# bacpop/sparrowhawk

Hardware: AMD Instinct MI355X
Metric: Gbases/s assembled, k=31 150bp reads (higher is better)
Workload: dtype u64

## Files before the change

sparrowhawk_amd/csrc/graph_part.h:

```cpp
#pragma once

struct MinScan {
    Nt32State first, last;
    uint32_t h_first, h_last;
    uint32_t min_wo_first;
    uint32_t min_wo_last;
    __device__ __forceinline__ uint32_t min_all() const { return min(min_wo_first, h_first); }
};

template <int W> __device__ __forceinline__ uint32_t km_base(const Kmer<W> &x, int k, int j) {
    return km_bits2<W>(x, 2 * (k - 1 - j));
}

template <int W> __device__ __forceinline__ MinScan km_min_scan(const Kmer<W> &x, int k, int gm) {
    MinScan r;
    Nt32State nt{0, 0};
    for (int j = 0; j < gm; j++) nt32_init_step(nt, km_base<W>(x, k, j), (unsigned)j);
    r.first = nt; r.h_first = nt32_canonical(nt);
    r.min_wo_first = 0xFFFFFFFFu; r.min_wo_last = r.h_first;
    const int w = k - gm + 1;
    uint32_t h = r.h_first;
    for (int q = 1; q < w; q++) {
        nt32_roll(nt, km_base<W>(x, k, q - 1), km_base<W>(x, k, q + gm - 1), (unsigned)gm);
        h = nt32_canonical(nt);
// ... 128 lines not shown
}

__global__ __launch_bounds__(1024) void k_gp_scan(uint32_t *__restrict__ gp_cnt , uint32_t GP,
                                                  unsigned long long *__restrict__ off, uint32_t *__restrict__ msk,
                                                  uint32_t *__restrict__ roff, unsigned long long *__restrict__ total) {
    constexpr uint32_t PER = 16, CH = 1024 * PER;
    __shared__ uint32_t lc[CH + CH / PER];
    __shared__ unsigned long long run_off[1024];
    __shared__ uint32_t run_roff[1024];
    __shared__ unsigned long long wsum[16];
    __shared__ uint32_t rsum[16];
    const int lane = threadIdx.x & 63, wid = threadIdx.x >> 6;
    unsigned long long carry = 0; uint32_t rcarry = 0;
    for (uint32_t c0 = 0; c0 < GP; c0 += CH) {
#pragma unroll
        for (uint32_t j = 0; j < PER; j++) {
            const uint32_t e = j * 1024u + threadIdx.x, p = c0 + e;
            lc[e + (e >> 4)] = p < GP ? gp_cnt[p] : 0u;
        }
#pragma unroll
        for (uint32_t j = 0; j < PER; j++) {
            const uint32_t p = c0 + j * 1024u + threadIdx.x;
            if (p < GP) gp_cnt[p] = 0u;
        }
        __syncthreads();
        unsigned long long my = 0; uint32_t myr = 0;
#pragma unroll
        for (uint32_t j = 0; j < PER; j++) {
            const uint32_t c = lc[threadIdx.x * (PER + 1u) + j];
            uint32_t sz = gp_table_size(c);
            if (c0 + threadIdx.x * PER + j >= GP) sz = 0;
            my += sz; myr += c;
        }
        unsigned long long incl = my; uint32_t rincl = myr;
        for (int o = 1; o < 64; o <<= 1) {
            const unsigned long long u = __shfl_up(incl, o); const uint32_t ru = (uint32_t)__shfl_up((int)rincl, o);
            if (lane >= o) { incl += u; rincl += ru; }
        }
        if (lane == 63) { wsum[wid] = incl; rsum[wid] = rincl; }
        __syncthreads();
        unsigned long long base = carry + incl - my; uint32_t rbase = rcarry + rincl - myr;
        for (int w = 0; w < wid; w++) { base += wsum[w]; rbase += rsum[w]; }
        run_off[threadIdx.x] = base; run_roff[threadIdx.x] = rbase;
        __syncthreads();
#pragma unroll 4
        for (uint32_t j = 0; j < PER; j++) {
            const uint32_t e = j * 1024u + threadIdx.x, p = c0 + e;
            const uint32_t c = lc[e + (e >> 4)];
            uint32_t sz = gp_table_size(c);
            if (p >= GP) sz = 0;
            uint32_t si = sz, ci = c;
#pragma unroll
            for (int o = 1; o < 16; o <<= 1) {
                const uint32_t u = (uint32_t)__shfl_up((int)si, o), v = (uint32_t)__shfl_up((int)ci, o);
                if ((lane & 15) >= o) { si += u; ci += v; }
            }
            if (p < GP) { off[p] = run_off[e >> 4] + (si - sz); msk[p] = sz - 1u; roff[p] = run_roff[e >> 4] + (ci - c); }
        }
        for (int w = 0; w < 16; w++) { carry += wsum[w]; rcarry += rsum[w]; }
        __syncthreads();
    }
    if (threadIdx.x == 0) { *total = carry; roff[GP] = rcarry; }
}

__global__ __launch_bounds__(256) void k_gp_rows(const uint32_t *__restrict__ gp_of, uint32_t n,
                                                 const uint32_t *__restrict__ roff, uint32_t *__restrict__ cursor,
                                                 uint32_t *__restrict__ rows) {
    const int lane = threadIdx.x & 63;
    const uint32_t stride = gridDim.x * blockDim.x;
    const uint32_t n_round = (n + stride - 1) / stride * stride;
    for (uint32_t i = blockIdx.x * blockDim.x + threadIdx.x; i < n_round; i += stride) {
        const uint32_t p = i < n ? gp_of[i] : 0xFFFFFFFFu;
        const bool valid = p != 0xFFFFFFFFu;
        unsigned long long todo = __ballot(valid);
        int my_leader = lane; uint32_t rank = 0, gsize = 0;
        while (todo) {
            const int leader = __ffsll((long long)todo) - 1;
            const uint32_t lp = (uint32_t)__shfl((int)p, leader);
            const unsigned long long same = __ballot(p == lp) & todo;
            if (valid && p == lp) { my_leader = leader; rank = (uint32_t)__popcll(same & ((1ull << lane) - 1ull)); gsize = (uint32_t)__popcll(same); }
            todo &= ~same;
        }
        const uint32_t ro = valid ? roff[p] : 0u;
        uint32_t base = 0;
        if (valid && lane == my_leader) base = atomicAdd(&cursor[p], gsize);
        base = (uint32_t)__shfl((int)base, my_leader);
        if (valid) rows[ro + base + rank] = i;
    }
}

template <int W>
__global__ __launch_bounds__(256) void k_regroup_rows(KeyArr<W> keys, const uint32_t *__restrict__ cnt, const uint32_t *__restrict__ gp_of,
                                                      uint32_t *__restrict__ rows, uint32_t n, KeyArr<W> out_keys,
                                                      uint32_t *__restrict__ out_cnt, uint32_t *__restrict__ out_gp_of) {
    for (uint32_t r = blockIdx.x * blockDim.x + threadIdx.x; r < n; r += gridDim.x * blockDim.x) {
        const uint32_t i = rows[r];
        out_keys.store(r, keys.load(i));
        out_cnt[r] = cnt[i];
        out_gp_of[r] = gp_of[i];
        rows[r] = r;
    }
}

template <int W>
__device__ __forceinline__ uint32_t gt_lookup_in(const GraphTable &gt, const KeyArr<W> &keys, const Kmer<W> &q,
                                                 uint32_t p) {
    const uint64_t h = gt_hash<W>(q);
    const uint32_t fp = (uint32_t)(h >> 32);
    const unsigned long long base = gt.off[p];
    const uint32_t mask = gt.msk[p];
    uint32_t slot = (uint32_t)h & mask;
    for (uint32_t t = 0; t <= mask; t++) {
        const uint64_t e = gt.e[base + slot];
        if (e == EMPTY64) return NIL;
        if ((uint32_t)(e >> 32) == fp) {
            const uint32_t idx = (uint32_t)e;
            if (km_eq<W>(keys.load(idx), q)) return idx;
        }
        slot = (slot + 1) & mask;
    }
    return NIL;
}
template <int W>
__device__ __forceinline__ uint32_t gt_lookup(const GraphTable &gt, const KeyArr<W> &keys, const Kmer<W> &q, int k) {
    return gt_lookup_in<W>(gt, keys, q, gt_partition_of<W>(gt, q, k));
}

static constexpr uint32_t ADJ_LDS_SLOTS = 2048;
static constexpr uint32_t NB_MULTI = 0xFFFFFFFEu;
static constexpr uint32_t ADJ_LDS_SLOTS_RANGES = 4096;
static constexpr int ADJ_THREADS_RANGES = 512;

struct GpRows {
    const uint32_t *roff;
    const uint32_t *cnt;
    const uint32_t *rows;
    __device__ __forceinline__ uint32_t begin(uint32_t P) const { return roff[P]; }
    __device__ __forceinline__ uint32_t end(uint32_t P) const { return cnt ? roff[P] + cnt[P] : roff[P + 1]; }
    __device__ __forceinline__ uint32_t row(uint32_t r) const { return rows ? rows[r] : r; }
};

template <int W>
__device__ __forceinline__ Kmer<W> adj_candidate(const Kmer<W> &x, const Kmer<W> &rx, int k, uint32_t j, bool &o) {
    Kmer<W> s = x, rr = rx;
    if (j < 4) { km_push_back<W>(s, j, k); km_push_front<W>(rr, 3u - j, k); }
    else { km_push_front<W>(s, j - 4u, k); km_push_back<W>(rr, 3u - (j - 4u), k); }
    o = km_less<W>(rr, s);
    Kmer<W> c;
#pragma unroll
    for (int w = 0; w < W; w++) c.w[w] = o ? rr.w[w] : s.w[w];
    return c;
}

template <int W, uint32_t SLOTS, int NT>
__global__ __launch_bounds__(NT) void k_graph_local(KeyArr<W> keys, int k, GraphTable gt, GpRows gr,
                                                    uint8_t *__restrict__ adj, uint32_t *__restrict__ nb,
                                                    unsigned long long *__restrict__ queries, uint32_t *__restrict__ qcnt,
                                                    uint32_t *__restrict__ overflow, uint32_t lds_slots ,
                                                    uint8_t *__restrict__ alive, uint32_t *__restrict__ row_bits, uint32_t lowmask) {
    const unsigned gm = (unsigned)gt.gm;
    __shared__ uint2 lut[16];
    __shared__ uint64_t tab[SLOTS];
    __shared__ uint32_t tabi[W == 1 ? SLOTS : 1];
    __shared__ uint32_t q_fill;
    const uint32_t P = blockIdx.x;
    const bool ranges = gr.cnt != nullptr;
    const uint32_t r0 = gr.begin(P), r1 = gr.end(P);
    const uint32_t pmask = gt.msk[P];
    const bool in_lds = pmask < lds_slots;
    uint64_t *gtab = gt.e + gt.off[P];
    nt32_fill_lut(lut, gm);
    const Nt32State all_a = nt32_all_a(gt.gm);
    if (threadIdx.x == 0) q_fill = 0;
    constexpr bool KEYS_IN_LDS = W == 1;
    for (uint32_t t = threadIdx.x; t <= pmask; t += blockDim.x) {
        if (in_lds) tab[t] = EMPTY64;
        if (!in_lds || KEYS_IN_LDS) gtab[t] = EMPTY64;
    }
    __syncthreads();
    constexpr int KEEP = 4;
    static_assert(SLOTS <= 2u * KEEP * NT, "a partition whose table fits the LDS keeps its rows in registers");
    const bool keep = W <= 2 && (r1 - r0) <= (uint32_t)KEEP * NT;
    static_assert(KEEP == 4, "kept rows are four named registers");
    const uint32_t rt = r0 + threadIdx.x;
    const uint32_t i0 = (keep && rt < r1) ? gr.row(rt) : NIL, i1 = (keep && rt + NT < r1) ? gr.row(rt + NT) : NIL;
    const uint32_t i2 = (keep && rt + 2 * NT < r1) ? gr.row(rt + 2 * NT) : NIL, i3 = (keep && rt + 3 * NT < r1) ? gr.row(rt + 3 * NT) : NIL;
    const Kmer<W> k0 = i0 != NIL ? keys.load(i0) : km_zero<W>(), k1 = i1 != NIL ? keys.load(i1) : km_zero<W>();
    const Kmer<W> k2 = i2 != NIL ? keys.load(i2) : km_zero<W>(), k3 = i3 != NIL ? keys.load(i3) : km_zero<W>();
    auto kept_i = [=](uint32_t q) { return q == 0 ? i0 : (q == 1 ? i1 : (q == 2 ? i2 : i3)); };
    auto kept_key = [=](uint32_t q) {
        Kmer<W> r;
#pragma unroll
        for (int w = 0; w < W; w++) r.w[w] = q == 0 ? k0.w[w] : (q == 1 ? k1.w[w] : (q == 2 ? k2.w[w] : k3.w[w]));
        return r;
    };
    for (uint32_t r = r0 + threadIdx.x, q = 0; r < r1; r += blockDim.x, q++) {
        const uint32_t i = keep ? kept_i(q) : gr.row(r);
        const Kmer<W> key = keep ? kept_key(q) : keys.load(i);
        const uint64_t h = gt_hash<W>(key);
        const uint64_t entry = (h & 0xFFFFFFFF00000000ull) | (uint64_t)i;
        uint32_t slot = (uint32_t)h & pmask;
        bool done = false;
        for (uint32_t t = 0; t <= pmask; t++) {
            if (in_lds && KEYS_IN_LDS) {
                if (atomicCAS((unsigned long long *)&tab[slot], (unsigned long long)EMPTY64, (unsigned long long)key.w[0]) == EMPTY64) {
                    tabi[slot] = i; gtab[slot] = entry; done = true; break;
                }
            } else {
                unsigned long long *cell = in_lds ? (unsigned long long *)&tab[slot] : (unsigned long long *)&gtab[slot];
                if (atomicCAS(cell, (unsigned long long)EMPTY64, (unsigned long long)entry) == EMPTY64) { done = true; break; }
            }
            slot = (slot + 1) & pmask;
        }
        if (!done) *overflow = 1;
    }
    __syncthreads();
    if (ranges && threadIdx.x == NT - 1 && r1 > r0) {
        bool st = r0 == 0u;
        if (!st) st = ((km_min_scan_lut<W>(keys.load(r0 - 1u), k, gt.gm, lut, all_a).min_all() ^ P) & lowmask) != 0u;
        if (st) atomicOr(&row_bits[r0 >> 5], 1u << (r0 & 31u));
    }
    if (in_lds && !KEYS_IN_LDS) for (uint32_t t = threadIdx.x; t <= pmask; t += blockDim.x) gtab[t] = tab[t];
    {
        uint8_t *occ = gt.occ + (gt.off[P] >> 3);
        for (uint32_t t8 = threadIdx.x; t8 <= (pmask >> 3); t8 += blockDim.x) {
            uint32_t bits = 0;
#pragma unroll
            for (uint32_t b = 0; b < 8; b++) {
                const uint64_t e = in_lds ? tab[8u * t8 + b] : __hip_atomic_load(&gtab[8u * t8 + b], __ATOMIC_RELAXED, __HIP_MEMORY_SCOPE_AGENT);
                bits |= (e != EMPTY64 ? 1u : 0u) << b;
            }
            occ[t8] = (uint8_t)bits;
        }
    }
    if (SHK_DBG(gt.dbg) == 1) { if (threadIdx.x == 0) qcnt[P] = 0; return; }
    unsigned long long *myq = queries + 8ull * r0;
    const int lane = threadIdx.x & 63;
    const uint32_t n_rows = r1 - r0;
    const uint32_t n_round = (n_rows + blockDim.x - 1) / blockDim.x * blockDim.x;
    for (uint32_t rr_ = threadIdx.x, q = 0; rr_ < n_round; rr_ += blockDim.x, q++) {
        const bool act = rr_ < n_rows;
        const uint32_t i = act ? (keep ? kept_i(q) : gr.row(r0 + rr_)) : 0u;
        Kmer<W> x = km_zero<W>(), rx = km_zero<W>();
        MinScan ms{};
        uint32_t out_b = 0, last_b = 0;
        if (act) {
            x = keep ? kept_key(q) : keys.load(i);
            rx = km_revcomp<W>(x, k);
            if (gt.scan) {
                const uint2 a = gt.scan[i], b = gt.scan[(size_t)gt.scan_n + i], c = gt.scan[2 * (size_t)gt.scan_n + i];
                ms.first.fh = a.x; ms.first.rh = a.y; ms.last.fh = b.x; ms.last.rh = b.y; ms.min_wo_first = c.x; ms.min_wo_last = c.y;
                ms.h_first = min(a.x, a.y); ms.h_last = min(b.x, b.y);
            } else
            if (SHK_DBG(gt.dbg) != 2) ms = km_min_scan_lut<W>(x, k, gt.gm, lut, all_a);
            if (ranges && ((ms.min_all() & gt.gp_mask) != P)) *overflow = 2u;
            out_b = km_base<W>(x, k, k - (int)gm);
            last_b = km_base<W>(x, k, (int)gm - 1);
        }
        uint32_t a = 0, n_out = 0, n_in = 0, u_out = NIL, u_in = NIL;
#pragma unroll
        for (uint32_t j = 0; j < 8; j++) {
            bool remote = false; uint32_t p = 0, xowner = 0; bool cross = false;
            if (act) {
                const uint32_t hmin = j < 4 ? min(ms.min_wo_first, nt32_next_hash_lut(ms.last, out_b, j, lut))
                                            : min(ms.min_wo_last, nt32_prev_hash_lut(ms.first, j - 4u, last_b, lut));
                p = hmin & gt.gp_mask;
                if (gt.world > 1) { xowner = gt.owner_of(hmin); cross = xowner != gt.rank; }
                remote = cross || p != P || !in_lds;
                if (SHK_DBG(gt.dbg) == 3) remote = false;
                if (SHK_DBG(gt.dbg) == 4 && remote) { remote = false; }
                else if (!remote && SHK_DBG(gt.dbg) != 3) {
                    bool o; const Kmer<W> c = adj_candidate<W>(x, rx, k, j, o);
                    const uint64_t h = gt_hash<W>(c);
                    const uint32_t fp = (uint32_t)(h >> 32);
                    uint32_t slot = (uint32_t)h & pmask, idx = NIL;
                    for (uint32_t t = 0; t <= pmask; t++) {
                        const uint64_t e = tab[slot];
                        if (e == EMPTY64) break;
                        if constexpr (KEYS_IN_LDS) { if (e == c.w[0]) { idx = tabi[slot]; break; } }
                        else if ((uint32_t)(e >> 32) == fp && km_eq<W>(keys.load((uint32_t)e), c)) { idx = (uint32_t)e; break; }
                        slot = (slot + 1) & pmask;
                    }
                    (void)fp;
                    if (idx != NIL) {
                        a |= 1u << j;
                        if (j < 4) { n_out++; u_out = idx * 2u + (o ? 1u : 0u); }
                        else { n_in++; u_in = idx * 2u + (o ? 0u : 1u); }
                    }
                }
            }
            const unsigned long long m = __ballot(remote);
            if (m) {
                uint32_t base = 0;
                if (lane == 0) base = atomicAdd(&q_fill, (uint32_t)__popcll(m));
                base = (uint32_t)__shfl((int)base, 0);
                if (remote) myq[base + (uint32_t)__popcll(m & ((1ull << lane) - 1ull))] =
                    (unsigned long long)i | ((unsigned long long)j << 32) | ((unsigned long long)p << 35) |
                    (cross ? (1ull << 63) | ((unsigned long long)xowner << 52) : 0ull);
            }
        }
        if (act) {
            adj[i] = (uint8_t)a;
            if (alive) alive[i] = 1;
            uint2 v;
            v.x = n_out == 0 ? NIL : (n_out == 1 ? u_out : NB_MULTI);
            v.y = n_in == 0 ? NIL : (n_in == 1 ? u_in : NB_MULTI);
            *reinterpret_cast<uint2 *>(nb + 2ull * i) = v;
        }
    }
    __syncthreads();
    if (threadIdx.x == 0) qcnt[P] = q_fill;
}

template <int W>
__global__ __launch_bounds__(256) void k_graph_remote(KeyArr<W> keys, int k, GraphTable gt, GpRows gr,
                                                      const unsigned long long *__restrict__ queries,
                                                      const uint32_t *__restrict__ qcnt,
                                                      uint8_t *__restrict__ adj, uint32_t *__restrict__ nb) {
    const uint32_t P = blockIdx.x;
    const unsigned long long *myq = queries + 8ull * gr.begin(P);
    const uint32_t nq = qcnt[P];
    constexpr int U = W <= 2 ? 4 : (W <= 4 ? 2 : 1);
    for (uint32_t t0 = threadIdx.x; t0 < nq; t0 += blockDim.x * U) {
        unsigned long long q[U]; bool live[U];
#pragma unroll
        for (int u = 0; u < U; u++) {
            const uint32_t t = t0 + (uint32_t)u * blockDim.x;
            q[u] = t < nq ? myq[t] : ~0ull;
            live[u] = !(q[u] >> 63);
        }
        Kmer<W> x[U]; unsigned long long tbase[U]; uint32_t tmask[U];
#pragma unroll
        for (int u = 0; u < U; u++) {
            const uint32_t i = (uint32_t)q[u], p = (uint32_t)(q[u] >> 35) & 0x1FFFFu;
            x[u] = live[u] ? keys.load(i) : km_zero<W>();
            tbase[u] = live[u] ? gt.off[p] : 0ull;
            tmask[u] = live[u] ? gt.msk[p] : 0u;
        }
        Kmer<W> c[U]; bool o[U]; uint32_t fp[U], slot[U]; uint64_t e[U];
#pragma unroll
        for (int u = 0; u < U; u++) {
            const uint32_t j = (uint32_t)(q[u] >> 32) & 7u;
            const Kmer<W> rx = km_revcomp<W>(x[u], k);
            c[u] = adj_candidate<W>(x[u], rx, k, j, o[u]);
            const uint64_t h = gt_hash<W>(c[u]);
            fp[u] = (uint32_t)(h >> 32); slot[u] = (uint32_t)h & tmask[u];
        }
        bool taken[U];
#pragma unroll
        for (int u = 0; u < U; u++) {
            const unsigned long long s = tbase[u] + slot[u];
            taken[u] = live[u] && ((gt.occ[s >> 3] >> (s & 7u)) & 1u);
        }
#pragma unroll
        for (int u = 0; u < U; u++) e[u] = taken[u] ? gt.e[tbase[u] + slot[u]] : EMPTY64;
        Kmer<W> cand[U]; bool want[U];
#pragma unroll
        for (int u = 0; u < U; u++) {
            want[u] = e[u] != EMPTY64 && (uint32_t)(e[u] >> 32) == fp[u];
            cand[u] = want[u] ? keys.load((uint32_t)e[u]) : km_zero<W>();
        }
#pragma unroll
        for (int u = 0; u < U; u++) {
            if (!live[u]) continue;
            uint32_t idx = NIL;
            if (want[u] && km_eq<W>(cand[u], c[u])) idx = (uint32_t)e[u];
            else if (e[u] != EMPTY64) {
                uint32_t s = (slot[u] + 1u) & tmask[u];
                for (uint32_t t = 1; t <= tmask[u]; t++) {
                    const uint64_t ee = gt.e[tbase[u] + s];
                    if (ee == EMPTY64) break;
                    if ((uint32_t)(ee >> 32) == fp[u] && km_eq<W>(keys.load((uint32_t)ee), c[u])) { idx = (uint32_t)ee; break; }
                    s = (s + 1u) & tmask[u];
                }
            }
            if (idx == NIL) continue;
            const uint32_t i = (uint32_t)q[u], j = (uint32_t)(q[u] >> 32) & 7u;
            atomicOr((uint32_t *)adj + (i >> 2), (1u << j) << (8 * (i & 3u)));
            const uint32_t v = j < 4 ? idx * 2u + (o[u] ? 1u : 0u) : idx * 2u + (o[u] ? 0u : 1u);
            uint32_t *dst = nb + 2ull * i + (j < 4 ? 0 : 1);
            if (atomicCAS(dst, NIL, v) != NIL) atomicExch(dst, NB_MULTI);
        }
    }
}

__device__ __forceinline__ uint32_t rev4(uint32_t n) {
    return ((n & 1) << 3) | ((n & 2) << 1) | ((n & 4) >> 1) | ((n & 8) >> 3);
}
__device__ __forceinline__ uint32_t outmask_of(uint32_t adjbyte, uint32_t o) {
    return o ? rev4(adjbyte >> 4) : (adjbyte & 15u);
}

template <int W> struct Graph {
    KeyArr<W> keys;
    const uint32_t *cnt;
    uint8_t *adj;
    GraphTable gt;
    const uint32_t *nb;
    int k;
    uint32_t n;
    uint32_t xref = 0;
    __device__ __forceinline__ uint32_t outmask(uint32_t v) const { return outmask_of(adj[v >> 1], v & 1); }
    __device__ __forceinline__ uint32_t outdeg(uint32_t v) const { return __popc(outmask(v)); }
    __device__ __forceinline__ uint32_t indeg(uint32_t v) const { return __popc(outmask(v ^ 1)); }
    __device__ __forceinline__ Kmer<W> seq(uint32_t v) const {
        Kmer<W> x = keys.load(v >> 1);
        return (v & 1) ? km_revcomp<W>(x, k) : x;
    }
    __device__ __forceinline__ uint32_t follow(uint32_t v, uint32_t b) const {
        Kmer<W> s = seq(v);
        km_push_back<W>(s, b, k);
        int o; Kmer<W> c = km_canonical<W>(s, k, o);
        uint32_t idx = gt_lookup<W>(gt, keys, c, k);
        return idx == NIL ? NIL : idx * 2 + (uint32_t)o;
    }
    __device__ __forceinline__ uint32_t only_out(uint32_t v) const {
        const uint32_t c = nb[v];
        if (c < NB_MULTI) return c;
        return follow(v, (uint32_t)__ffs((int)outmask(v)) - 1);
    }
};

struct TipRec { uint32_t start, junction, len, next; unsigned long long sum; };

template <int W>
__global__ __launch_bounds__(256) void k_tip_candidates(Graph<W> g, const uint8_t *__restrict__ alive,
                                                        uint32_t *__restrict__ cand,
                                                        unsigned int *__restrict__ n_cand,
                                                        uint2 *__restrict__ init_tip_head ,
                                                        uint8_t *__restrict__ init_mark ) {
    const int lane = threadIdx.x & 63;
    const uint32_t stride = gridDim.x * blockDim.x;
    const uint32_t n_round = (g.n + stride - 1) / stride * stride;
    for (uint32_t i = blockIdx.x * blockDim.x + threadIdx.x; i < n_round; i += stride) {
        uint32_t a = 0; bool al = false;
        if (i < g.n) {
            a = g.adj[i]; al = alive[i] != 0;
            if (init_tip_head) { uint2 nil; nil.x = NIL; nil.y = NIL; init_tip_head[i] = nil; init_mark[i] = 0; }
        }
#pragma unroll
        for (uint32_t o = 0; o < 2; o++) {
            const bool p = al && __popc(outmask_of(a, o ^ 1u)) == 0 && __popc(outmask_of(a, o)) == 1;
            const unsigned long long m = __ballot(p);
            if (!m) continue;
            unsigned int base = 0;
            if (lane == 0) base = atomicAdd(n_cand, (unsigned int)__popcll(m));
            base = __shfl(base, 0);
            if (p) cand[base + __popcll(m & ((1ull << lane) - 1ull))] = 2u * i + o;
        }
    }
}

template <int W>
__global__ __launch_bounds__(256) void k_tip_walk(Graph<W> g, const uint32_t *__restrict__ cand,
                                                  const unsigned int *__restrict__ n_cand_p, TipRec *__restrict__ tips,
                                                  unsigned int *__restrict__ n_tips,
                                                  uint32_t *__restrict__ tip_head) {
    const uint32_t T_TIP = 2u * (uint32_t)g.k;
    const uint32_t n_cand = *n_cand_p;
    for (uint32_t c = blockIdx.x * blockDim.x + threadIdx.x; c < n_cand; c += gridDim.x * blockDim.x) {
        const uint32_t v = cand[c];
        uint32_t cur = v, len = 1, J = NIL;
        unsigned long long sum = g.cnt[v >> 1];
        uint32_t a_cur = g.adj[cur >> 1], nb_cur = g.nb[cur];
        for (;;) {
            const uint32_t om = outmask_of(a_cur, cur & 1u);
            if (__popc(om) != 1) break;
            const uint32_t n = nb_cur < NB_MULTI ? nb_cur : g.follow(cur, (uint32_t)__ffs((int)om) - 1u);
            if (n == NIL) break;
            const uint32_t a_n = g.adj[n >> 1], nb_n = g.nb[n], c_n = g.cnt[n >> 1];
            if (__popc(outmask_of(a_n, (n & 1u) ^ 1u)) >= 2) { J = n; break; }
            len++; sum += c_n; cur = n; a_cur = a_n; nb_cur = nb_n;
            if (len > T_TIP) break;
        }
        if (J == NIL || len > T_TIP) continue;
        const uint32_t t = atomicAdd(n_tips, 1u);
        TipRec r; r.start = v; r.junction = J; r.len = len; r.sum = sum;
        r.next = atomicExch(&tip_head[J], t);
        tips[t] = r;
    }
}

template <int W>
__global__ __launch_bounds__(256) void k_tip_decide(Graph<W> g, const TipRec *__restrict__ tips,
                                                    const unsigned int *__restrict__ n_tips_p,
                                                    const uint32_t *__restrict__ tip_head,
                                                    uint8_t *__restrict__ kill) {
    const uint32_t n_tips = *n_tips_p;
    for (uint32_t a = blockIdx.x * blockDim.x + threadIdx.x; a < n_tips; a += gridDim.x * blockDim.x) {
        const TipRec me = tips[a];
        const uint32_t d = g.indeg(me.junction);
        uint32_t t = 0; bool best = true;
        const Kmer<W> myfirst = g.keys.load(me.start >> 1);
        for (uint32_t b = tip_head[me.junction]; b != NIL; b = tips[b].next) {
            t++;
            if (b == a) continue;
            const TipRec o = tips[b];
            bool better;
            if (o.len != me.len) better = o.len > me.len;
            else if (o.sum != me.sum) better = o.sum > me.sum;
            else better = km_less<W>(g.keys.load(o.start >> 1), myfirst);
            if (better) best = false;
        }
        kill[a] = (t < d) ? 1 : (best ? 0 : 1);
    }
}

template <int W>
__global__ __launch_bounds__(256) void k_tip_remove(Graph<W> g, const TipRec *__restrict__ tips,
                                                    const unsigned int *__restrict__ n_tips_p, const uint8_t *__restrict__ kill,
                                                    uint32_t *__restrict__ tip_head,
                                                    uint8_t *__restrict__ mark) {
    const uint32_t n_tips = *n_tips_p;
    for (uint32_t a = blockIdx.x * blockDim.x + threadIdx.x; a < n_tips; a += gridDim.x * blockDim.x) {
        const TipRec me = tips[a];
        if (kill[a]) {
            uint32_t cur = me.start;
            for (uint32_t i = 0; i < me.len; i++) {
                mark[cur >> 1] = 1;
                if (i + 1 < me.len) cur = g.only_out(cur);
            }
        }
    }
}

__global__ __launch_bounds__(256) void k_tip_reset_heads(const TipRec *__restrict__ tips, const unsigned int *__restrict__ n_tips_p,
                                                         uint32_t *__restrict__ tip_head) {
    const uint32_t n_tips = *n_tips_p;
    for (uint32_t a = blockIdx.x * blockDim.x + threadIdx.x; a < n_tips; a += gridDim.x * blockDim.x)
        tip_head[tips[a].junction] = NIL;
}

template <int W>
__global__ __launch_bounds__(256) void k_fork_candidates(Graph<W> g, const uint8_t *__restrict__ alive,
// ... 141 lines not shown
```

sparrowhawk_amd/csrc/pipeline.hip:

```cpp
#include <hip/hip_runtime.h>
#include <hipcub/hipcub.hpp>
#include <thread>
#include <stdint.h>
#include <stdio.h>
#include <stdlib.h>
#include <string.h>
#include <algorithm>
#include <atomic>
#include <chrono>
#include <map>
#include <memory>
#include <mutex>
#include <string>
#include <vector>

#include "kmer.h"
#include "pipeline.h"
#include "shard_comm.h"
#include "unitig_graph.h"

namespace shk {

#define HIPCHK(call)                                                                      \
    do {                                                                                  \
// ... 1160 lines not shown
                           (OvfRec *)nullptr, (uint32_t *)nullptr, 0u, 0u, (uint32_t *)nullptr);
        HIPCHK(hipGetLastError());
        t.mark();
        std::vector<uint32_t> h(pp_.P);
        HIPCHK(hipMemcpyAsync(h.data(), dd_n_.p, (size_t)pp_.P * 4, hipMemcpyDeviceToHost, stream_));
        WAIT_STREAM();
        times_.add("shard_dedupe_kernel", t.elapsed());
        unsigned long long n_dd = 0;
        for (uint32_t p = 0; p < pp_.P; p++) { part_records[p] = h[p]; n_dd += h[p]; }
        times_.add("shard_dedupe_records_in_x1e-6", (double)n_raw * 1e-6);
        times_.add("shard_dedupe_records_out_x1e-6", (double)n_dd * 1e-6);
        have_dedup_ = true;
        return 0;
    }
    void shard_drop_dedup() override { dd_recs_.release(); dd_w_.release(); dd_base_.release(); dd_n_.release(); have_dedup_ = false; }
    int shard_pack_dedup(void *d_send, void *d_send_w, const uint64_t *base_records, uint32_t n_partitions, std::string &err) override {
        if (!have_dedup_) return 0;
        if (n_partitions != pp_.P) { err = "partition count mismatch"; return -1; }
        DevBuf<unsigned long long> base;
        if (int rc = base.alloc(pp_.P, err)) return rc;
        HIPCHK(hipMemcpyAsync(base.p, base_records, (size_t)pp_.P * 8, hipMemcpyHostToDevice, stream_));
        EvTimer t(stream_, stage_timers_);
        hipLaunchKernelGGL((k_pack_dedup<2 * W>), dim3(pp_.P), dim3(256), 0, stream_, dd_recs_.p, dd_w_.p, dd_base_.p, dd_n_.p, base.p,
                           (uint64_t *)d_send, (uint32_t *)d_send_w);
        HIPCHK(hipGetLastError());
        if (t.on()) times_.add("shard_pack_kernel", t.stop());
        WAIT_STREAM();
        shard_drop_dedup();
        recs_.release(); fill_.release(); run_off_.release(); run_cnt_.release(); have_parts_ = false;
        return 0;
    }

    int shard_count(const void *d_recv, const void *d_recv_w, const uint64_t *run_off, const uint32_t *run_cnt, uint32_t n_owned,
                    uint32_t n_sources, uint32_t emit_threshold, uint64_t histo[500], std::string &err) override {
        if (n_sources < 1 || n_sources > 256) { err = "1..256 sources"; return -1; }
        const uint64_t n_runs = (uint64_t)n_owned * n_sources;
        if (int rc = run_off_.alloc(n_runs, err)) return rc;
        if (int rc = run_cnt_.alloc(n_runs, err)) return rc;
        std::vector<unsigned long long> addr16(n_runs);
        for (uint64_t i = 0; i < n_runs; i++) addr16[i] = ((unsigned long long)(uintptr_t)d_recv >> 4) + run_off[i] * (unsigned long long)W;
        if (n_runs) {
            HIPCHK(hipMemcpyAsync(run_off_.p, addr16.data(), n_runs * 8, hipMemcpyHostToDevice, stream_));
            HIPCHK(hipMemcpyAsync(run_cnt_.p, run_cnt, n_runs * 4, hipMemcpyHostToDevice, stream_));
        }
        shard_recv_ = d_recv;
        run_view_.run_addr16 = run_off_.p; run_view_.run_cnt = run_cnt_.p;
        run_view_.S = n_sources; run_view_.k = k_; n_count_parts_ = n_owned; run_view_.dbg = 0;
        run_view_.weights = (const uint32_t *)d_recv_w; run_view_.rec_base16 = (unsigned long long)(uintptr_t)d_recv >> 4;
        uint64_t total_recs = 0;
        for (uint32_t j = 0; j < n_owned; j++) {
            uint64_t r = 0;
            for (uint32_t s = 0; s < n_sources; s++) r += run_cnt[(uint64_t)j * n_sources + s];
            if (r > 0xFFFFFFF0ull) { err = "a partition holds more than 2^32 records"; return -1; }
            total_recs += r;
        }
        memset(histo, 0, 500 * 8);
        n_emitted_ = 0; emit_threshold_ = emit_threshold; n_distinct_ = 0;
        double ms = 0; uint64_t inst = 0;
        have_parts_ = n_runs != 0;
        const uint64_t rows_hint = d_recv_w ? 2 * total_recs + (1u << 16) : std::max<uint64_t>(1u << 16, total_recs);
        if (int rc = run_count_partitions(run_view_, n_owned, emit_threshold, ekeys_, ecnt_, n_emitted_, histo, inst,
                                          rows_hint, ms, err)) return rc;
        times_.add("count_kernel", ms);
        total_instances_ = inst;
        for (int i = 0; i < 500; i++) { histo_[i] = histo[i]; n_distinct_ += histo[i]; }
        return 0;
    }

    int shard_rows(uint32_t threshold, const void **keys_soa, const void **cnt, uint64_t *n, std::string &err) override {
        if (int rc = filter(threshold, err)) return rc;
        for (int j = 0; j < W; j++) keys_soa[j] = skeys_[j].p;
        *cnt = scnt_.p; *n = n_solid_;
        return 0;
    }

    int shard_set_solid(const void *const *keys_soa, const void *cnt, uint64_t n, const uint64_t histo[500],
                        uint64_t total_instances, std::string &err) override {
        if (n >= 0x7FFFFFFFull) { err = "too many solid k-mers for 32-bit node ids"; return -1; }
        DevBuf<uint64_t> nk[W]; DevBuf<uint32_t> nc;
        for (int j = 0; j < W; j++) {
            if (int rc = nk[j].alloc(n, err)) return rc;
            if (n) HIPCHK(hipMemcpyAsync(nk[j].p, keys_soa[j], n * 8, hipMemcpyDeviceToDevice, stream_));
        }
        if (int rc = nc.alloc(n, err)) return rc;
        if (n) HIPCHK(hipMemcpyAsync(nc.p, cnt, n * 4, hipMemcpyDeviceToDevice, stream_));
        WAIT_STREAM();
        for (int j = 0; j < W; j++) skeys_[j].swap(nk[j]);
        scnt_.swap(nc);
        n_solid_ = n; total_instances_ = total_instances; n_distinct_ = 0; er_ok_ = false;
        for (int i = 0; i < 500; i++) { histo_[i] = histo[i]; n_distinct_ += histo[i]; }
        graph_ready_ = false;
        return 0;
    }

    Graph<W> graph_view() {
        Graph<W> g;
        for (int j = 0; j < W; j++) g.keys.w[j] = skeys_[j].p;
        g.cnt = scnt_.p; g.adj = adj_.p; g.nb = nb_.p; g.k = k_;
        g.gt.e = gt_.p; g.gt.occ = gt_occ_.p; g.gt.scan = gt_scan_.p; g.gt.scan_n = gt_scan_.p ? (uint32_t)n_solid_ : 0u; g.gt.off = gt_off_.p; g.gt.msk = gt_msk_.p; g.gt.gp_mask = gp_ - 1u; g.gt.gm = part_m(k_); g.gt.dbg = env_dbg("SHK_DEBUG_G");
        g.n = (uint32_t)n_solid_;
        if (sh_active_) {
            g.gt.cp_mask = sh_P_ - 1u; g.gt.world = sh_world_; g.gt.rank = sh_rank_;
            g.gt.world_inv = (uint32_t)((0x100000000ull + sh_world_ - 1u) / sh_world_);
            g.xref = XREF;
        }
        return g;
    }

    int build_graph(std::string &err) override {
        const uint64_t n = n_solid_;
        for (int j = 0; j < W; j++) tkeys_[j].release();
        tcnt_.release(); tstate_.release(); tslots_ = 0;
        recs_.release(); fill_.release(); run_off_.release(); run_cnt_.release(); shard_recv_ = nullptr; batches_.clear();
        const uint64_t regroup_env = env_u64("SHK_REGROUP_ROWS", 2);
        const uint64_t range_rows = env_u64("SHK_GRAPH_RANGE_ROWS", ADJ_LDS_SLOTS_RANGES * 3 / 8);
        const bool ranges = er_ok_ && er_rows_ == n && n && !sh_active_ && !rows_scattered_ && regroup_env != 1 &&
                            n <= (uint64_t)er_groups_ * range_rows &&
                            getenv("SHK_GP_ROWS") == nullptr && env_u64("SHK_GRAPH_RANGES", 1) != 0;
        er_ok_ = false;
        gp_ = 64;
        const uint64_t gp_rows_target = env_u64("SHK_GP_ROWS", 640);
        const uint64_t n_for_gp = sh_active_ ? n_solid_global_ : n;
        while (gp_ < GP_MAX && (uint64_t)gp_ * gp_rows_target < n_for_gp) gp_ <<= 1;
        if (ranges) gp_ = er_groups_;
        gt_slots_ = 4 * n + 8ull * gp_;
        if (int rc = gt_.alloc(gt_slots_, err)) return rc;
        if (int rc = gt_occ_.alloc(gt_slots_ / 8 + 8, err)) return rc;
        gt_scan_.release();
        if (!ranges && n && n <= (64ull << 20) && env_u64("SHK_KEEP_SCAN", 1)) if (int rc = gt_scan_.alloc(3 * n, err)) return rc;
        DevBuf<uint32_t> gp_of, gp_cnt, gp_roff, gp_rows, gp_n;
        if (ranges) {
            gt_off_.swap(er_off_); gt_msk_.swap(er_msk_); gp_roff.swap(er_start_); gp_n.swap(er_cnt_);
            er_off_.release(); er_msk_.release(); er_start_.release(); er_cnt_.release();
        } else {
            if (int rc = gt_off_.alloc(gp_, err)) return rc;
            if (int rc = gt_msk_.alloc(gp_, err)) return rc;
            if (int rc = gp_of.alloc(n, err)) return rc;
            if (int rc = gp_roff.alloc(gp_ + 1, err)) return rc;
            if (int rc = gp_rows.alloc(n, err)) return rc;
        }
        if (int rc = gp_cnt.alloc(gp_, err)) return rc;
        DevBuf<unsigned long long> queries;
        if (int rc = queries.alloc(8 * n + 8, err)) return rc;
        if (int rc = adj_.alloc((n + 8) & ~3ull, err)) return rc;
        if (keep_stages_) if (int rc = adj0_.alloc(n, err)) return rc;
        if (int rc = nb_.alloc(2 * n + 2, err)) return rc;
        if (int rc = alive_.alloc(n, err)) return rc;
        if (int rc = row_starts_.alloc(((n + 63) / 64) * 2 + 2, err)) return rc;
        if (ranges) HIPCHK(fill2_async(row_starts_.p, row_starts_.bytes, 0u, ctl_.p, CTL_WORDS * sizeof(unsigned long long), 0u, stream_));
        else HIPCHK(fill2_async(gp_cnt.p, (size_t)gp_ * 4, 0u, ctl_.p, CTL_WORDS * sizeof(unsigned long long), 0u, stream_));
        if (n || sh_active_) {
            Graph<W> g = graph_view();
            const uint32_t lowmask = std::min<uint32_t>(gp_, 256u) - 1u;
            if (ranges) {
                EvTimer t(stream_, stage_timers_);
                t.stop_later("graph_table_kernel", pending_timers_);
                EvTimer t2(stream_, stage_timers_);
                const GpRows gr{gp_roff.p, gp_n.p, nullptr};
                const uint32_t lds_slots = (uint32_t)std::min<uint64_t>(env_u64("SHK_GRAPH_LDS_SLOTS", ADJ_LDS_SLOTS_RANGES), ADJ_LDS_SLOTS_RANGES);
                hipLaunchKernelGGL((k_graph_local<W, ADJ_LDS_SLOTS_RANGES, ADJ_THREADS_RANGES>), dim3(gp_), dim3(ADJ_THREADS_RANGES), 0, stream_,
                                   g.keys, k_, g.gt, gr, adj_.p, nb_.p, queries.p, gp_cnt.p, (uint32_t *)(ctl_.p + 1), lds_slots,
                                   alive_.p, row_starts_.p, lowmask);
                hipLaunchKernelGGL(k_graph_remote<W>, dim3(gp_), dim3(256), 0, stream_, g.keys, k_, g.gt, gr, queries.p,
                                   gp_cnt.p, adj_.p, nb_.p);
                HIPCHK(hipGetLastError());
                t2.stop_later("adjacency_kernel", pending_timers_);
                times_.add("graph_partitions_from_counting_x1", 1.0);
            } else {
                EvTimer t(stream_, stage_timers_);
                hipLaunchKernelGGL(k_gp_count<W>, dim3(grid_for(n)), dim3(256), 0, stream_, g.keys, (uint32_t)n, k_, g.gt,
                                   gp_of.p, gp_cnt.p);
                hipLaunchKernelGGL(k_gp_scan, dim3(1), dim3(1024), 0, stream_, gp_cnt.p, gp_, gt_off_.p, gt_msk_.p, gp_roff.p,
                                   ctl_.p + 2);
                hipLaunchKernelGGL(k_gp_rows, dim3(grid_for(n)), dim3(256), 0, stream_, gp_of.p, (uint32_t)n, gp_roff.p, gp_cnt.p,
                                   gp_rows.p);
                HIPCHK(hipGetLastError());
                if (n && (regroup_env == 1 || (regroup_env == 2 && rows_scattered_))) {
                    DevBuf<uint64_t> nk[W]; DevBuf<uint32_t> nc, ngp;
                    for (int j = 0; j < W; j++) if (int rc = nk[j].alloc(n, err)) return rc;
                    if (int rc = nc.alloc(n, err)) return rc;
                    if (int rc = ngp.alloc(n, err)) return rc;
                    KeyArr<W> out_keys; for (int j = 0; j < W; j++) out_keys.w[j] = nk[j].p;
                    hipLaunchKernelGGL(k_regroup_rows<W>, dim3(grid_for(n)), dim3(256), 0, stream_, g.keys, scnt_.p, gp_of.p, gp_rows.p, (uint32_t)n,
                                       out_keys, nc.p, ngp.p);
                    HIPCHK(hipGetLastError());
                    WAIT_STREAM();
                    for (int j = 0; j < W; j++) skeys_[j].swap(nk[j]);
                    scnt_.swap(nc); gp_of.swap(ngp);
                    gt_scan_.release();
                    g = graph_view();
                    times_.add("graph_rows_regrouped_x1", 1.0);
                }
                hipLaunchKernelGGL(k_row_starts, dim3(grid_for(n)), dim3(256), 0, stream_, gp_of.p, (uint32_t)n, lowmask,
                                   row_starts_.p, alive_.p);
                t.stop_later("graph_table_kernel", pending_timers_);
                EvTimer t2(stream_, stage_timers_);
                const GpRows gr{gp_roff.p, nullptr, gp_rows.p};
                hipLaunchKernelGGL((k_graph_local<W, ADJ_LDS_SLOTS, 256>), dim3(gp_), dim3(256), 0, stream_, g.keys, k_, g.gt, gr,
                                   adj_.p, nb_.p, queries.p, gp_cnt.p, (uint32_t *)(ctl_.p + 1), ADJ_LDS_SLOTS,
                                   (uint8_t *)nullptr, (uint32_t *)nullptr, 0u);
                hipLaunchKernelGGL(k_graph_remote<W>, dim3(gp_), dim3(256), 0, stream_, g.keys, k_, g.gt, gr, queries.p,
                                   gp_cnt.p, adj_.p, nb_.p);
                HIPCHK(hipGetLastError());
                t2.stop_later("adjacency_kernel", pending_timers_);
                times_.add("graph_partitions_cut_x1", 1.0);
            }
            if (sh_active_ && sh_world_ > 1) {
                HIPCHK(fill2_async(ctl_.p + 13, 8, 0u, nullptr, 0, 0u, stream_));
                hipLaunchKernelGGL(k_xq_total, dim3(gp_), dim3(256), 0, stream_, gp_roff.p, queries.p, gp_cnt.p, (unsigned int *)(ctl_.p + 13));
                unsigned int n_x = 0;
                if (int rc = read_ctl(n_x, 13, err)) return rc;
                xq_n_ = n_x;
                if (int rc = xq_dest_.alloc(n_x, err)) return rc;
                if (int rc = xq_pay_.alloc((size_t)n_x * (W + 1), err)) return rc;
                if (int rc = xq_meta_.alloc(n_x, err)) return rc;
                if (n_x) {
                    HIPCHK(fill2_async(ctl_.p + 13, 8, 0u, nullptr, 0, 0u, stream_));
                    hipLaunchKernelGGL(k_xq_stage<W>, dim3(gp_), dim3(256), 0, stream_, g.keys, k_, gp_roff.p, queries.p, gp_cnt.p,
                                       (unsigned int *)(ctl_.p + 13), n_x, xq_dest_.p, xq_pay_.p, xq_meta_.p);
                    HIPCHK(hipGetLastError());
                }
            }
            if (keep_stages_) HIPCHK(hipMemcpyAsync(adj0_.p, adj_.p, n, hipMemcpyDeviceToDevice, stream_));
            graph_check_pending_ = true;
            if (sh_active_) {
                HIPCHK(hipMemcpyAsync(mbox64() + MB_CTL, ctl_.p, 3 * 8, hipMemcpyDeviceToHost, stream_));
                WAIT_STREAM();
                if (int rc = check_graph_flags(err)) return rc;
            }
            if (!sh_active_ || sh_world_ <= 1) {  }
        }
        graph_ready_ = true;
        return 0;
    }

    int check_graph_flags(std::string &err) {
        if (!graph_check_pending_) return 0;
        graph_check_pending_ = false;
        const unsigned long long *h = mbox64() + MB_CTL;
        if ((uint32_t)h[1] == 2u) { err = "graph partition: a row lies outside its counting group's minimiser range"; return -6; }
        if ((uint32_t)h[1] || h[2] > gt_slots_) { err = "graph table overflow"; return -6; }
        return 0;
    }
    int read_ctl(unsigned int &v, int slot, std::string &err) {
        unsigned long long h = 0;
        HIPCHK(hipMemcpyAsync(&h, ctl_.p + slot, 8, hipMemcpyDeviceToHost, stream_));
        WAIT_STREAM();
        v = (unsigned int)h;
        return 0;
    }

    int apply_marks(Graph<W> &g, DevBuf<uint8_t> &mark, DevBuf<uint32_t> &removed, int slot, std::string &err) {
        const uint32_t n = (uint32_t)n_solid_;
        hipLaunchKernelGGL(k_collect_marked, dim3(grid_for(n)), dim3(256), 0, stream_, n, mark.p, alive_.p,
                           removed.p, (unsigned int *)(ctl_.p + slot));
        hipLaunchKernelGGL(k_apply_removed<W>, dim3(1024), dim3(256), 0, stream_, g, removed.p,
                           (const unsigned int *)(ctl_.p + slot));
        HIPCHK(hipGetLastError());
        return 0;
    }

    int correct(bool tips, bool bubbles, std::string &err) override {
        if (!graph_ready_) { err = "graph not built"; return -2; }
        const uint32_t n = (uint32_t)n_solid_;
        tips_removed_ = bubbles_removed_ = 0; rounds_ = 0;
        corr_pending_ = false; corr_tips_ = tips; corr_bubbles_ = bubbles;
        if (n == 0 || (!tips && !bubbles)) return 0;
        if (int rc = corr_.cand.alloc(2ull * n, err)) return rc;
        if (int rc = corr_.removed.alloc(n, err)) return rc;
        if (int rc = corr_.mark.alloc(n, err)) return rc;
        if (!tips) HIPCHK(hipMemsetAsync(corr_.mark.p, 0, n, stream_));
        if (tips) {
            if (int rc = corr_.tip_head.alloc(2ull * n, err)) return rc;
            if (int rc = corr_.tiprec.alloc(2ull * n, err)) return rc;
            if (int rc = corr_.kill.alloc(2ull * n, err)) return rc;
        }
        EvTimer t(stream_, stage_timers_);
        if (int rc = correction_round(0, err)) return rc;
        t.stop_later("correct_total", pending_timers_);
        corr_pending_ = true;
        return 0;
    }
    struct CorrScratch { DevBuf<uint32_t> cand, tip_head, removed; DevBuf<uint8_t> mark, kill; DevBuf<TipRec> tiprec;
                         void release() { cand.release(); tip_head.release(); removed.release(); mark.release(); kill.release(); tiprec.release(); } };
    int correction_round(int round, std::string &err) {
        const uint32_t n = (uint32_t)n_solid_;
        Graph<W> g = graph_view();
        const dim3 G(1024), B(256);
        const bool tips = corr_tips_, bubbles = corr_bubbles_;
        const int s_tip = round == 0 ? 16 : 5, s_bub = round == 0 ? 17 : 6;
        HIPCHK(fill2_async(ctl_.p + 3, 4 * 8, 0u, nullptr, 0, 0u, stream_));
        if (tips) {
            hipLaunchKernelGGL(k_tip_candidates<W>, dim3(grid_for(n)), B, 0, stream_, g, alive_.p,
                               corr_.cand.p, (unsigned int *)(ctl_.p + 3), round == 0 ? (uint2 *)corr_.tip_head.p : (uint2 *)nullptr,
                               round == 0 ? corr_.mark.p : (uint8_t *)nullptr);
            hipLaunchKernelGGL(k_tip_walk<W>, G, B, 0, stream_, g, corr_.cand.p, (const unsigned int *)(ctl_.p + 3),
                               corr_.tiprec.p, (unsigned int *)(ctl_.p + 4), corr_.tip_head.p);
            hipLaunchKernelGGL(k_tip_decide<W>, G, B, 0, stream_, g, corr_.tiprec.p, (const unsigned int *)(ctl_.p + 4),
                               corr_.tip_head.p, corr_.kill.p);
            hipLaunchKernelGGL(k_tip_remove<W>, G, B, 0, stream_, g, corr_.tiprec.p, (const unsigned int *)(ctl_.p + 4),
                               corr_.kill.p, corr_.tip_head.p, corr_.mark.p);
            hipLaunchKernelGGL(k_tip_reset_heads, G, B, 0, stream_, corr_.tiprec.p, (const unsigned int *)(ctl_.p + 4),
                               corr_.tip_head.p);
            HIPCHK(hipGetLastError());
            if (int rc = apply_marks(g, corr_.mark, corr_.removed, s_tip, err)) return rc;
        }
        if (bubbles) {
            HIPCHK(fill2_async(ctl_.p + 3, 8, 0u, nullptr, 0, 0u, stream_));
            hipLaunchKernelGGL(k_fork_candidates<W>, dim3(grid_for(n)), B, 0, stream_, g, alive_.p,
                               corr_.cand.p, (unsigned int *)(ctl_.p + 3));
            hipLaunchKernelGGL(k_bubble<W>, G, B, 0, stream_, g, corr_.cand.p, (const unsigned int *)(ctl_.p + 3), corr_.mark.p);
            HIPCHK(hipGetLastError());
            if (int rc = apply_marks(g, corr_.mark, corr_.removed, s_bub, err)) return rc;
        }
        return 0;
    }
    int finish_correction(unsigned int n1, unsigned int n2, std::string &err) {
        corr_pending_ = false;
        tips_removed_ += n1; bubbles_removed_ += n2; rounds_ = 1;
        EvTimer t(stream_, stage_timers_);
        for (int round = 1; round < 32 && n1 + n2 != 0; round++) {
            if (int rc = correction_round(round, err)) return rc;
            HIPCHK(hipMemcpyAsync(mbox64() + MB_MISC, ctl_.p + 5, 16, hipMemcpyDeviceToHost, stream_));
            WAIT_STREAM();
            n1 = (unsigned int)mbox64()[MB_MISC]; n2 = (unsigned int)mbox64()[MB_MISC + 1];
            tips_removed_ += n1; bubbles_removed_ += n2; rounds_++;
        }
        if (rounds_ > 1) if (t.on()) times_.add("correct_total", t.stop());
        corr_.release();
        return 0;
    }

    int get_adjacency(uint8_t *adj_initial, uint8_t *adj_final, uint8_t *alive, uint64_t cap,
                      std::string &err) override {
        if (!graph_ready_) { err = "graph not built"; return -2; }
        if (cap < n_solid_) { err = "buffer too small"; return -1; }
        if (!n_solid_) return 0;
        if (adj_initial && !keep_stages_) { err = "the initial adjacency is kept for inspection only on a verbose handle (or with SHK_KEEP_STAGES=1)"; return -2; }
        if (adj_initial) HIPCHK(hipMemcpy(adj_initial, adj0_.p, n_solid_, hipMemcpyDeviceToHost));
        if (adj_final) HIPCHK(hipMemcpy(adj_final, adj_.p, n_solid_, hipMemcpyDeviceToHost));
        if (alive) HIPCHK(hipMemcpy(alive, alive_.p, n_solid_, hipMemcpyDeviceToHost));
        return 0;
    }

    struct ChainState {
        DevBuf<uint32_t> spl, slot_of;
        DevBuf<uint2> winfo, ol;
        DevBuf<SegRec> segs;
        DevBuf<FragRec> frag;
        DevBuf<RankRec> Ra, Rb;
        DevBuf<FinRec> fin;
        DevBuf<HeadRec> d_heads;
        DevBuf<RingMin> ringmin;
        std::vector<HeadRec> heads;
        uint32_t seg_cap = 0;
// ... 1011 lines not shown
```

Before: 176.2.

## Probe each de Bruijn edge once and mirror it to the neighbour

Adds a HALF variant of the local and remote adjacency kernels, on by default when not sharded. Each k-mer now probes only the neighbours whose canonical form is not smaller than its own, and writes the mirrored edge bit and unique-neighbour code into the other endpoint. Rows are accumulated in an LDS word using 16-bit local row indices and flushed after a barrier. The aim is to roughly halve the hash probes and candidate work, at the cost of extra LDS atomics, global atomicOr/CAS on adj and nb for remote edges, and an extra LDS array plus a row-count limit on LDS partitions.

```diff
diff --git a/sparrowhawk_amd/csrc/graph_part.h b/sparrowhawk_amd/csrc/graph_part.h
--- a/sparrowhawk_amd/csrc/graph_part.h
+++ b/sparrowhawk_amd/csrc/graph_part.h
@@ -304,7 +304,18 @@
     return c;
 }
 
-template <int W, uint32_t SLOTS, int NT>
+struct Mirror { uint32_t bit, side, orient; };
+__device__ __forceinline__ Mirror mirror_of(uint32_t j, bool o, uint32_t f, uint32_t l) {
+    Mirror m;
+    if (j < 4) { m.bit = o ? 3u - f : 4u + f; m.side = o ? 0u : 1u; m.orient = 1u; }
+    else { m.bit = o ? 7u - l : l; m.side = o ? 1u : 0u; m.orient = 0u; }
+    return m;
+}
+struct RowWord {
+    static constexpr uint32_t ROWS_MAX = 2048;
+    static __device__ __forceinline__ uint32_t field(uint32_t side, uint32_t code) { return code << (side ? 20 : 8); }
+};
+template <int W, uint32_t SLOTS, int NT, bool HALF>
 __global__ __launch_bounds__(NT) void k_graph_local(KeyArr<W> keys, int k, GraphTable gt, GpRows gr,
                                                     uint8_t *__restrict__ adj, uint32_t *__restrict__ nb,
                                                     unsigned long long *__restrict__ queries, uint32_t *__restrict__ qcnt,
@@ -313,13 +324,16 @@
     const unsigned gm = (unsigned)gt.gm;
     __shared__ uint2 lut[16];
     __shared__ uint64_t tab[SLOTS];
-    __shared__ uint32_t tabi[W == 1 ? SLOTS : 1];
+    typedef typename std::conditional<HALF, uint16_t, uint32_t>::type TabI;
+    __shared__ TabI tabi[(W == 1 || HALF) ? SLOTS : 1];
+    __shared__ uint32_t roww[HALF ? SLOTS / 2 : 1];
+    static_assert(!HALF || SLOTS / 2 <= RowWord::ROWS_MAX, "a row's place inside the partition takes 11 bits");
     __shared__ uint32_t q_fill;
     const uint32_t P = blockIdx.x;
     const bool ranges = gr.cnt != nullptr;
     const uint32_t r0 = gr.begin(P), r1 = gr.end(P);
     const uint32_t pmask = gt.msk[P];
-    const bool in_lds = pmask < lds_slots;
+    const bool in_lds = pmask < lds_slots && (!HALF || r1 - r0 <= SLOTS / 2);
     uint64_t *gtab = gt.e + gt.off[P];
     nt32_fill_lut(lut, gm);
     const Nt32State all_a = nt32_all_a(gt.gm);
@@ -329,6 +343,7 @@
         if (in_lds) tab[t] = EMPTY64;
         if (!in_lds || KEYS_IN_LDS) gtab[t] = EMPTY64;
     }
+    if (HALF && in_lds) for (uint32_t t = threadIdx.x; t < r1 - r0; t += blockDim.x) roww[t] = 0u;
     __syncthreads();
     constexpr int KEEP = 4;
     static_assert(SLOTS <= 2u * KEEP * NT, "a partition whose table fits the LDS keeps its rows in registers");
@@ -356,11 +371,14 @@
         for (uint32_t t = 0; t <= pmask; t++) {
             if (in_lds && KEYS_IN_LDS) {
                 if (atomicCAS((unsigned long long *)&tab[slot], (unsigned long long)EMPTY64, (unsigned long long)key.w[0]) == EMPTY64) {
-                    tabi[slot] = i; gtab[slot] = entry; done = true; break;
+                    tabi[slot] = (TabI)(HALF ? r - r0 : i); gtab[slot] = entry; done = true; break;
                 }
             } else {
                 unsigned long long *cell = in_lds ? (unsigned long long *)&tab[slot] : (unsigned long long *)&gtab[slot];
-                if (atomicCAS(cell, (unsigned long long)EMPTY64, (unsigned long long)entry) == EMPTY64) { done = true; break; }
+                if (atomicCAS(cell, (unsigned long long)EMPTY64, (unsigned long long)entry) == EMPTY64) {
+                    if (HALF && in_lds) tabi[slot] = (TabI)(r - r0);
+                    done = true; break;
+                }
             }
             slot = (slot + 1) & pmask;
         }
@@ -395,7 +413,7 @@
         const uint32_t i = act ? (keep ? kept_i(q) : gr.row(r0 + rr_)) : 0u;
         Kmer<W> x = km_zero<W>(), rx = km_zero<W>();
         MinScan ms{};
-        uint32_t out_b = 0, last_b = 0;
+        uint32_t out_b = 0, last_b = 0, first_x = 0, last_x = 0;
         if (act) {
             x = keep ? kept_key(q) : keys.load(i);
             rx = km_revcomp<W>(x, k);
@@ -408,21 +426,24 @@
             if (ranges && ((ms.min_all() & gt.gp_mask) != P)) *overflow = 2u;
             out_b = km_base<W>(x, k, k - (int)gm);
             last_b = km_base<W>(x, k, (int)gm - 1);
-        }
-        uint32_t a = 0, n_out = 0, n_in = 0, u_out = NIL, u_in = NIL;
+            first_x = km_first_base<W>(x, k); last_x = km_last_base<W>(x);
+        }
+        uint32_t a = 0, n_out = 0, n_in = 0, u_out = HALF ? 0u : NIL, u_in = HALF ? 0u : NIL;
 #pragma unroll
         for (uint32_t j = 0; j < 8; j++) {
             bool remote = false; uint32_t p = 0, xowner = 0; bool cross = false;
-            if (act) {
+            bool o = false; Kmer<W> c = km_zero<W>(); bool mine = act;
+            if constexpr (HALF) if (act) { c = adj_candidate<W>(x, rx, k, j, o); mine = !km_less<W>(c, x); }
+            if (mine) {
                 const uint32_t hmin = j < 4 ? min(ms.min_wo_first, nt32_next_hash_lut(ms.last, out_b, j, lut))
                                             : min(ms.min_wo_last, nt32_prev_hash_lut(ms.first, j - 4u, last_b, lut));
                 p = hmin & gt.gp_mask;
-                if (gt.world > 1) { xowner = gt.owner_of(hmin); cross = xowner != gt.rank; }
+                if (!HALF && gt.world > 1) { xowner = gt.owner_of(hmin); cross = xowner != gt.rank; }
                 remote = cross || p != P || !in_lds;
                 if (SHK_DBG(gt.dbg) == 3) remote = false;
                 if (SHK_DBG(gt.dbg) == 4 && remote) { remote = false; }
                 else if (!remote && SHK_DBG(gt.dbg) != 3) {
-                    bool o; const Kmer<W> c = adj_candidate<W>(x, rx, k, j, o);
+                    if constexpr (!HALF) c = adj_candidate<W>(x, rx, k, j, o);
                     const uint64_t h = gt_hash<W>(c);
                     const uint32_t fp = (uint32_t)(h >> 32);
                     uint32_t slot = (uint32_t)h & pmask, idx = NIL;
@@ -430,14 +451,22 @@
                         const uint64_t e = tab[slot];
                         if (e == EMPTY64) break;
                         if constexpr (KEYS_IN_LDS) { if (e == c.w[0]) { idx = tabi[slot]; break; } }
-                        else if ((uint32_t)(e >> 32) == fp && km_eq<W>(keys.load((uint32_t)e), c)) { idx = (uint32_t)e; break; }
+                        else if ((uint32_t)(e >> 32) == fp && km_eq<W>(keys.load((uint32_t)e), c)) { idx = HALF ? (uint32_t)tabi[slot] : (uint32_t)e; break; }
                         slot = (slot + 1) & pmask;
                     }
                     (void)fp;
                     if (idx != NIL) {
                         a |= 1u << j;
+                        if constexpr (HALF) {
+                            if (j < 4) u_out |= idx * 2u + (o ? 1u : 0u); else u_in |= idx * 2u + (o ? 0u : 1u);
+                            if (idx != rr_) {
+                                const Mirror m = mirror_of(j, o, first_x, last_x);
+                                atomicOr(&roww[idx], (1u << m.bit) | RowWord::field(m.side, rr_ * 2u + m.orient));
+                            }
+                        } else {
                         if (j < 4) { n_out++; u_out = idx * 2u + (o ? 1u : 0u); }
                         else { n_in++; u_in = idx * 2u + (o ? 0u : 1u); }
+                        }
                     }
                 }
             }
@@ -451,6 +480,9 @@
                     (cross ? (1ull << 63) | ((unsigned long long)xowner << 52) : 0ull);
             }
         }
+        if (HALF && in_lds) {
+            if (act) atomicOr(&roww[rr_], a | RowWord::field(0, u_out) | RowWord::field(1, u_in));
+        } else
         if (act) {
             adj[i] = (uint8_t)a;
             if (alive) alive[i] = 1;
@@ -461,10 +493,23 @@
         }
     }
     __syncthreads();
+    if (HALF && in_lds)
+        for (uint32_t rr_ = threadIdx.x, q = 0; rr_ < n_rows; rr_ += blockDim.x, q++) {
+            const uint32_t i = keep ? kept_i(q) : gr.row(r0 + rr_);
+            const uint32_t w = roww[rr_];
+            const uint32_t n_out = __popc(w & 15u), n_in = __popc(w & 0xF0u);
+            const uint32_t c_out = (w >> 8) & 0xFFFu, c_in = w >> 20;
+            adj[i] = (uint8_t)w;
+            if (alive) alive[i] = 1;
+            uint2 v;
+            v.x = n_out == 0 ? NIL : (n_out == 1 ? gr.row(r0 + (c_out >> 1)) * 2u + (c_out & 1u) : NB_MULTI);
+            v.y = n_in == 0 ? NIL : (n_in == 1 ? gr.row(r0 + (c_in >> 1)) * 2u + (c_in & 1u) : NB_MULTI);
+            *reinterpret_cast<uint2 *>(nb + 2ull * i) = v;
+        }
     if (threadIdx.x == 0) qcnt[P] = q_fill;
 }
 
-template <int W>
+template <int W, bool HALF>
 __global__ __launch_bounds__(256) void k_graph_remote(KeyArr<W> keys, int k, GraphTable gt, GpRows gr,
                                                       const unsigned long long *__restrict__ queries,
                                                       const uint32_t *__restrict__ qcnt,
@@ -532,6 +577,12 @@
             const uint32_t v = j < 4 ? idx * 2u + (o[u] ? 1u : 0u) : idx * 2u + (o[u] ? 0u : 1u);
             uint32_t *dst = nb + 2ull * i + (j < 4 ? 0 : 1);
             if (atomicCAS(dst, NIL, v) != NIL) atomicExch(dst, NB_MULTI);
+            if (HALF && idx != i) {
+                const Mirror m = mirror_of(j, o[u], km_first_base<W>(x[u], k), km_last_base<W>(x[u]));
+                atomicOr((uint32_t *)adj + (idx >> 2), (1u << m.bit) << (8 * (idx & 3u)));
+                uint32_t *mdst = nb + 2ull * idx + m.side;
+                if (atomicCAS(mdst, NIL, i * 2u + m.orient) != NIL) atomicExch(mdst, NB_MULTI);
+            }
         }
     }
 }
diff --git a/sparrowhawk_amd/csrc/pipeline.hip b/sparrowhawk_amd/csrc/pipeline.hip
--- a/sparrowhawk_amd/csrc/pipeline.hip
+++ b/sparrowhawk_amd/csrc/pipeline.hip
@@ -1336,17 +1336,21 @@
         if (n || sh_active_) {
             Graph<W> g = graph_view();
             const uint32_t lowmask = std::min<uint32_t>(gp_, 256u) - 1u;
+            const bool half = !sh_active_ && env_u64("SHK_GRAPH_HALF", 1) != 0;
+            times_.add(half ? "graph_probe_half_x1" : "graph_probe_full_x1", 1.0);
             if (ranges) {
                 EvTimer t(stream_, stage_timers_);
                 t.stop_later("graph_table_kernel", pending_timers_);
                 EvTimer t2(stream_, stage_timers_);
                 const GpRows gr{gp_roff.p, gp_n.p, nullptr};
                 const uint32_t lds_slots = (uint32_t)std::min<uint64_t>(env_u64("SHK_GRAPH_LDS_SLOTS", ADJ_LDS_SLOTS_RANGES), ADJ_LDS_SLOTS_RANGES);
-                hipLaunchKernelGGL((k_graph_local<W, ADJ_LDS_SLOTS_RANGES, ADJ_THREADS_RANGES>), dim3(gp_), dim3(ADJ_THREADS_RANGES), 0, stream_,
+                auto local = half ? k_graph_local<W, ADJ_LDS_SLOTS_RANGES, ADJ_THREADS_RANGES, true>
+                                  : k_graph_local<W, ADJ_LDS_SLOTS_RANGES, ADJ_THREADS_RANGES, false>;
+                hipLaunchKernelGGL(local, dim3(gp_), dim3(ADJ_THREADS_RANGES), 0, stream_,
                                    g.keys, k_, g.gt, gr, adj_.p, nb_.p, queries.p, gp_cnt.p, (uint32_t *)(ctl_.p + 1), lds_slots,
                                    alive_.p, row_starts_.p, lowmask);
-                hipLaunchKernelGGL(k_graph_remote<W>, dim3(gp_), dim3(256), 0, stream_, g.keys, k_, g.gt, gr, queries.p,
-                                   gp_cnt.p, adj_.p, nb_.p);
+                hipLaunchKernelGGL((half ? k_graph_remote<W, true> : k_graph_remote<W, false>), dim3(gp_), dim3(256), 0, stream_,
+                                   g.keys, k_, g.gt, gr, queries.p, gp_cnt.p, adj_.p, nb_.p);
                 HIPCHK(hipGetLastError());
                 t2.stop_later("adjacency_kernel", pending_timers_);
                 times_.add("graph_partitions_from_counting_x1", 1.0);
@@ -1380,11 +1384,12 @@
                 t.stop_later("graph_table_kernel", pending_timers_);
                 EvTimer t2(stream_, stage_timers_);
                 const GpRows gr{gp_roff.p, nullptr, gp_rows.p};
-                hipLaunchKernelGGL((k_graph_local<W, ADJ_LDS_SLOTS, 256>), dim3(gp_), dim3(256), 0, stream_, g.keys, k_, g.gt, gr,
+                auto local = half ? k_graph_local<W, ADJ_LDS_SLOTS, 256, true> : k_graph_local<W, ADJ_LDS_SLOTS, 256, false>;
+                hipLaunchKernelGGL(local, dim3(gp_), dim3(256), 0, stream_, g.keys, k_, g.gt, gr,
                                    adj_.p, nb_.p, queries.p, gp_cnt.p, (uint32_t *)(ctl_.p + 1), ADJ_LDS_SLOTS,
                                    (uint8_t *)nullptr, (uint32_t *)nullptr, 0u);
-                hipLaunchKernelGGL(k_graph_remote<W>, dim3(gp_), dim3(256), 0, stream_, g.keys, k_, g.gt, gr, queries.p,
-                                   gp_cnt.p, adj_.p, nb_.p);
+                hipLaunchKernelGGL((half ? k_graph_remote<W, true> : k_graph_remote<W, false>), dim3(gp_), dim3(256), 0, stream_,
+                                   g.keys, k_, g.gt, gr, queries.p, gp_cnt.p, adj_.p, nb_.p);
                 HIPCHK(hipGetLastError());
                 t2.stop_later("adjacency_kernel", pending_timers_);
                 times_.add("graph_partitions_cut_x1", 1.0);
```

Result: no change. 178.7 (median of 6 runs) (+1.4%).
